# superxslam/SuperOdom

Measured on AMD Instinct MI355X. Metric: icp_registrations_per_sec, higher is better.
Workload: dtype f64

## Files before the change

superodom_amd/csrc/kernels.hip:

```cpp
#include <hip/hip_runtime.h>
#include <hip/hip_ext.h>

#include <cstddef>
#include <cstdlib>
#include <cstring>
#include <type_traits>

#ifdef SO_LM_STAMPS
#define SO_LM_STAMP(dbg, i) do { if (dbg) (dbg)[i] = wall_clock64(); } while (0)
#endif
#include "device_idioms.h"
#include "kernels.h"
#include "plane_fit.h"

namespace soicp {

#define SO_MATCH_SUCCESS 0
#define SO_MATCH_NOT_ENOUGH 1
#define SO_MATCH_TOO_FAR 2
#define SO_MATCH_BAD_PCA 3
#define SO_MATCH_INVALID 4
#define SO_MATCH_MSE 5
#define SO_MATCH_DROPPED 254
#define SO_MATCH_PENDING 255
// ... 1547 lines not shown
}
__device__ __forceinline__ void publish_state_to(DevState* dst, const DevState* st, unsigned long long seq, int tid, int nthreads) {
  if (!dst) return;
  __threadfence_block();
  __syncthreads();
  const unsigned long long* src = reinterpret_cast<const unsigned long long*>(st);
  unsigned long long* out = reinterpret_cast<unsigned long long*>(dst);
  constexpr int kWords = (int)(offsetof(DevState, seq) / 8);
  for (int i = tid; i < kWords; i += nthreads) out[i] = src[i];
  __threadfence_system();
  __syncthreads();
  if (tid == 0) __hip_atomic_store(&dst->seq, seq, __ATOMIC_RELEASE, __HIP_MEMORY_SCOPE_SYSTEM);
}

__device__ __forceinline__ void copy_words(double* dst, const double* src, int n_doubles, int tid, int nthreads) {
  for (int i = tid; i < n_doubles; i += nthreads) dst[i] = src[i];
}
static_assert(sizeof(LmState) % 8 == 0 && sizeof(LmSums) % 8 == 0, "controller state must be double-aligned");

constexpr int kPartStride = SO_SOLVE_BLOCKS;
static_assert(kEvalBlocks <= kPartStride && kFitBlocksMax <= kPartStride && kNAcc <= kSumsStride, "partials table");
constexpr int kRedStride = kNAcc + 2;

template <int CTRL>
__device__ __forceinline__ double dpp_f64(double v) {
  const int lo = __builtin_amdgcn_update_dpp(0, __double2loint(v), CTRL, 0xF, 0xF, false);
  const int hi = __builtin_amdgcn_update_dpp(0, __double2hiint(v), CTRL, 0xF, 0xF, false);
  return __hiloint2double(hi, lo);
}
__device__ __forceinline__ double swap32_add(double a, double b) {
  const auto lo = __builtin_amdgcn_permlane32_swap((unsigned)__double2loint(a), (unsigned)__double2loint(b), false, false);
  const auto hi = __builtin_amdgcn_permlane32_swap((unsigned)__double2hiint(a), (unsigned)__double2hiint(b), false, false);
  return __hiloint2double((int)hi[0], (int)lo[0]) + __hiloint2double((int)hi[1], (int)lo[1]);
}
__device__ __forceinline__ double swap16_add(double a, double b) {
  const auto lo = __builtin_amdgcn_permlane16_swap((unsigned)__double2loint(a), (unsigned)__double2loint(b), false, false);
  const auto hi = __builtin_amdgcn_permlane16_swap((unsigned)__double2hiint(a), (unsigned)__double2hiint(b), false, false);
  return __hiloint2double((int)hi[0], (int)lo[0]) + __hiloint2double((int)hi[1], (int)lo[1]);
}
template <int CTRL>
__device__ __forceinline__ double row_stage_add(double a, double b, bool up) {
  const double keep = up ? b : a, give = up ? a : b;
  return keep + dpp_f64<CTRL>(give);
}
__device__ __forceinline__ double wave_reduce_scatter(const double (&acc)[kNAcc]) {
  static_assert(kNAcc > 16 && kNAcc <= 32, "butterfly over 32 value slots");
  const int lane = (int)(threadIdx.x & 63u);
  double u[16], w[8], x[4], y[2];
#pragma unroll
  for (int a = 0; a < 16; ++a) u[a] = swap32_add(acc[a], (a + 16 < kNAcc) ? acc[a + 16] : 0.0);
#pragma unroll
  for (int a = 0; a < 8; ++a) w[a] = swap16_add(u[a], u[a + 8]);
  const bool b3 = (lane & 8) != 0, b2 = (lane & 4) != 0, b1 = (lane & 2) != 0;
#pragma unroll
  for (int a = 0; a < 4; ++a) x[a] = row_stage_add<0x128>(w[a], w[a + 4], b3);
#pragma unroll
  for (int a = 0; a < 2; ++a) y[a] = row_stage_add<0x141>(x[a], x[a + 2], b2);
  const double z = row_stage_add<0x4E>(y[0], y[1], b1);
  return z + dpp_f64<0xB1>(z);
}
__device__ __forceinline__ double wg_reduce(const double (&acc)[kNAcc], double (*part)[32], int tid) {
  const double t = wave_reduce_scatter(acc);
  const int lane = tid & 63, wave = tid >> 6;
  if (!(lane & 1) && (lane >> 1) < kNAcc) part[wave][lane >> 1] = t;
  __syncthreads();
  double tot = 0;
  if (tid < kNAcc) tot = ((part[0][tid] + part[1][tid]) + part[2][tid]) + part[3][tid];
  return tot;
}

__device__ __forceinline__ double reduce_records(double (*red)[kRedStride], double (*part)[32], int tid) {
  const int a = tid & 31, cch = tid >> 5;
  if (a < kNAcc) {
    double s = 0;
#pragma unroll 8
    for (int r = 0; r < 32; ++r) s += red[cch * 32 + r][a];
    part[cch][a] = s;
  }
  __syncthreads();
  double tot = 0;
  if (tid < kNAcc) {
#pragma unroll
    for (int cc = 0; cc < 8; ++cc) tot += part[cc][tid];
  }
  return tot;
}

struct EvalShared {
  double red[256][kRedStride];
  double part[8][32];
  double part_odd[8][32];
  LmSums sums;
  LmState S;
  LmCtl ctl;
  double pose[7];
  int more;
  int32_t lh[16];
  int32_t hpart[8][16];
  int reg_done;
  bool is_last;
  unsigned long long peer_seq;
};
struct CorrCache {
  double nx[2][256], ny[2][256], nz[2][256], nw[2][256], c[2][256];
  float px[2][256], py[2][256], pz[2][256];
};
enum { kPassNotLast = 0, kPassMore = 1, kPassDone = 2, kPassSums = 3 };

struct WgSpan { uint32_t vb0, vb1, V; bool ctl; };
template <bool FIT, bool PERSIST = false, bool PROF = false, bool BATCH = false, bool PEER = false>
__device__ __forceinline__ int eval_pass(int slot, int fuse_lm, const Pose& pose, const float* __restrict__ spx,
                                         const float* __restrict__ spy, const float* __restrict__ spz,
                                         const CorrBuffers& corr, DevState* __restrict__ st, const EvalParams& ep,
                                         double* __restrict__ partials, uint32_t* __restrict__ ticket,
                                         int32_t* __restrict__ hist, LmSums* __restrict__ out,
                                         const float4* __restrict__ mpts, const uint32_t* __restrict__ nbr5,
                                         const MatchParams& mp, EvalShared& sh, unsigned long long pass_tag = 0,
                                         CorrCache* cc = nullptr, u4v* hand = nullptr, unsigned long long want = 0,
                                         const WgSpan span = WgSpan{0, 0, 0, false}) {
  constexpr bool keep_state = PERSIST;
  double (*red)[kRedStride] = sh.red;
  double (*part)[32] = sh.part;
  LmSums& sh_sums = sh.sums;
  LmState& sh_S = sh.S;
  LmCtl& sh_ctl = sh.ctl;
  int& sh_more = sh.more;
  int32_t* lh = sh.lh;
  bool& is_last = sh.is_last;
  const int tid = threadIdx.x;
  static_assert(!BATCH || PERSIST, "batched hypotheses run in the persistent solve launch");
  const int abl = PROF ? ep.ablate : 0;
  const bool stamp = PROF && (abl & 128) != 0;
  const uint32_t V = BATCH ? span.V : gridDim.x;
  const uint32_t vb_begin = BATCH ? span.vb0 : blockIdx.x, vb_end = BATCH ? span.vb1 : blockIdx.x + 1u;
  const bool is_ctl = BATCH ? span.ctl : (blockIdx.x == 0);
  unsigned long long t_begin = 0, t_loop = 0, t_red = 0, t_ticket = 0, t_loaded = 0, t_sums = 0, t_lm = 0;
  if (stamp) t_begin = wall_clock64();
  if (FIT) {
    if (tid < 16) lh[tid] = 0;
    __syncthreads();
  }
  const uint32_t n_kept = (abl & 64) ? 0u : ep.n_queries;
  const uint32_t qs = ep.q_stride;
  double acc[kNAcc];
  const double qx = pose.q[0], qy = pose.q[1], qz = pose.q[2], qw = pose.q[3];
  const double tx = 2 * qx, ty = 2 * qy, tz = 2 * qz;
  const double twx = tx * qw, twy = ty * qw, twz = tz * qw, txx = tx * qx, txy = ty * qx, txz = tz * qx;
  const double tyy = ty * qy, tyz = tz * qy, tzz = tz * qz;
  const double R00 = 1 - (tyy + tzz), R01 = txy - twz, R02 = txz + twy;
  const double R10 = txy + twz, R11 = 1 - (txx + tzz), R12 = tyz - twx;
  const double R20 = txz - twy, R21 = tyz + twx, R22 = 1 - (txx + tyy);
  const ObsAxes axes = obs_axes(pose);
  const double inv_a2 = 1.0 / ep.a2, rho_out = (ep.variant == 0) ? ep.a2 / 6.0 : ep.a2 / 3.0;
  auto tail = [&](double px, double py, double pz, double wx, double wy, double wz, const double4& nd, double c) {
    const double r = SO_FMA(nd.x, wx, SO_FMA(nd.y, wy, SO_FMA(nd.z, wz, nd.w)));
    const double s = r * r;
    double rho0, rho1;
    if (s <= ep.a2) {
      const double v = 1.0 - s * inv_a2, v2 = v * v;
      rho0 = rho_out * (1.0 - v2 * v); rho1 = (ep.variant == 0) ? 0.5 * v2 : v2;
    } else {
      rho0 = rho_out; rho1 = 0;
    }
    const double w = c * rho1;
    const double m0 = SO_FMA(R00, nd.x, SO_FMA(R10, nd.y, R20 * nd.z));
    const double m1 = SO_FMA(R01, nd.x, SO_FMA(R11, nd.y, R21 * nd.z));
    const double m2 = SO_FMA(R02, nd.x, SO_FMA(R12, nd.y, R22 * nd.z));
    const double J[6] = {nd.x, nd.y, nd.z, SO_FMA(py, m2, -(pz * m1)), SO_FMA(pz, m0, -(px * m2)), SO_FMA(px, m1, -(py * m0))};
    acc[0] = SO_FMA(0.5 * c, rho0, acc[0]);
    acc[1] += 1.0;
    const double wr = w * r;
    int k = 8;
#pragma unroll
    for (int a = 0; a < 6; ++a) {
      acc[2 + a] = SO_FMA(J[a], wr, acc[2 + a]);
      const double wj = w * J[a];
#pragma unroll
      for (int b = a; b < 6; ++b) { acc[k] = SO_FMA(wj, J[b], acc[k]); ++k; }
    }
  };
  auto body = [&](const uint32_t j, int status, const float* nb, int trip) {
    if (!FIT && status != SO_MATCH_SUCCESS) return;
    if (FIT && status == SO_MATCH_DROPPED) return;
    const float fx = spx[(size_t)j * qs], fy = spy[(size_t)j * qs], fz = spz[(size_t)j * qs];
    const double px = (double)fx, py = (double)fy, pz = (double)fz;
    double wx, wy, wz;
    quat_rotate<double>(pose.q, px, py, pz, wx, wy, wz);
    wx += pose.t[0]; wy += pose.t[1]; wz += pose.t[2];
    double c;
    double4 nd;
    if (FIT) {
      if (PERSIST && !BATCH && trip >= 0) {
        cc->px[trip][tid] = fx; cc->py[trip][tid] = fy; cc->pz[trip][tid] = fz;
      }
      double fnd[4] = {0, 0, 0, 0}, fc = 0;
      int obs[3] = {0, 0, 0};
      if (status == SO_MATCH_PENDING) {
        const double pw[3] = {wx, wy, wz};
        if (PROF && (mp.ablate & (512 | 4096))) status = plane_fit5_reference(nb, pw, axes, mp.sq_max_dist_f, mp.max_point_dist, fnd, fc, obs, (mp.ablate & 512) != 0);
        else status = plane_fit5(nb, pw, axes, mp.sq_max_dist_f, mp.max_point_dist, fnd, fc, obs);
      }
      if (status != SO_MATCH_SUCCESS) { fc = 0; fnd[0] = fnd[1] = fnd[2] = fnd[3] = 0; }
      nd = make_double4(fnd[0], fnd[1], fnd[2], fnd[3]);
      c = fc;
      __builtin_nontemporal_store(nd.x, &corr.nd[j].x); __builtin_nontemporal_store(nd.y, &corr.nd[j].y);
      __builtin_nontemporal_store(nd.z, &corr.nd[j].z); __builtin_nontemporal_store(nd.w, &corr.nd[j].w);
      __builtin_nontemporal_store(c, &corr.coeff[j]); __builtin_nontemporal_store((uint8_t)status, &corr.status[j]);
      atomicAdd(&lh[status], 1);
      if (status == SO_MATCH_SUCCESS) { atomicAdd(&lh[7 + obs[0]], 1); atomicAdd(&lh[7 + obs[1]], 1); atomicAdd(&lh[7 + obs[2]], 1); }
      if (status != SO_MATCH_SUCCESS) return;
      if (PERSIST && !BATCH && trip >= 0) {
        cc->nx[trip][tid] = nd.x; cc->ny[trip][tid] = nd.y; cc->nz[trip][tid] = nd.z; cc->nw[trip][tid] = nd.w;
        cc->c[trip][tid] = c;
      }
    } else {
      c = corr.coeff[j];
      nd = corr.nd[j];
    }
    tail(px, py, pz, wx, wy, wz, nd, c);
  };
  double mine = 0;
  u4v* rec = reinterpret_cast<u4v*>(partials);
  const unsigned int tag = (unsigned int)pass_tag;
  struct Fetched { int st; double4 nd; double c; float x, y, z; };
  Fetched cur[2], nxt[2];
  auto fetch2 = [&](uint32_t vb_, Fetched (&o)[2]) {
#pragma unroll
    for (int q = 0; q < 2; ++q) {
      const uint32_t j = query_of(vb_, V, tid, (uint32_t)q);
      const uint32_t js = j < n_kept ? j : 0u;
      o[q].st = j < n_kept ? (int)corr.status[js] : (int)SO_MATCH_DROPPED;
      o[q].nd = corr.nd[js]; o[q].c = corr.coeff[js];
      o[q].x = spx[(size_t)js * qs]; o[q].y = spy[(size_t)js * qs]; o[q].z = spz[(size_t)js * qs];
    }
  };
  if (BATCH && !FIT && vb_begin < vb_end) fetch2(vb_begin, cur);
  for (uint32_t vb = vb_begin, trip_ = 0; BATCH ? (vb < vb_end) : (trip_ < 1u); ++vb, ++trip_) {
#pragma unroll
  for (int a = 0; a < kNAcc; ++a) acc[a] = 0;
  if (FIT) {
    if (PERSIST && !BATCH) { cc->c[0][tid] = -1.0; cc->c[1][tid] = -1.0; }
    bool first = true;
    if (BATCH) {
      for (uint32_t q = 0, j; (j = query_of(vb, V, tid, q)) < n_kept; ++q) {
        const int stq = corr.status[j];
        uint32_t iq[5];
#pragma unroll
        for (int t = 0; t < 5; ++t) iq[t] = nbr5[(size_t)5 * j + t];
        float nbq[15];
#pragma unroll
        for (int t = 0; t < 5; ++t) {
          const float4 a = mpts[stq == SO_MATCH_PENDING ? iq[t] : 0u];
          nbq[3 * t] = a.x; nbq[3 * t + 1] = a.y; nbq[3 * t + 2] = a.z;
        }
        body(j, stq, nbq, -1);
      }
    } else
    for (uint32_t q = 0, jA; (jA = query_of(vb, V, tid, q)) < n_kept; q += 2) {
      const uint32_t jB = query_of(vb, V, tid, q + 1u);
      const bool hasB = jB < n_kept;
      const uint32_t jBs = hasB ? jB : jA;
      const int stA = corr.status[jA];
      const int stB = hasB ? (int)corr.status[jBs] : SO_MATCH_NOT_ENOUGH;
      uint32_t iA[5], iB[5];
#pragma unroll
      for (int t = 0; t < 5; ++t) { iA[t] = nbr5[(size_t)5 * jA + t]; iB[t] = nbr5[(size_t)5 * jBs + t]; }
      float nbA[15], nbB[15];
#pragma unroll
      for (int t = 0; t < 5; ++t) {
        const float4 a = mpts[stA == SO_MATCH_PENDING ? iA[t] : 0u], b = mpts[stB == SO_MATCH_PENDING ? iB[t] : 0u];
        nbA[3 * t] = a.x; nbA[3 * t + 1] = a.y; nbA[3 * t + 2] = a.z;
        nbB[3 * t] = b.x; nbB[3 * t + 1] = b.y; nbB[3 * t + 2] = b.z;
      }
      body(jA, stA, nbA, first ? 0 : -1);
      if (hasB) body(jB, stB, nbB, first ? 1 : -1);
      first = false;
    }
  } else if (PERSIST && !BATCH) {
#pragma unroll
    for (int trip = 0; trip < 2; ++trip) {
      const double c = cc->c[trip][tid];
      const double4 nd = make_double4(cc->nx[trip][tid], cc->ny[trip][tid], cc->nz[trip][tid], cc->nw[trip][tid]);
      const double px = (double)cc->px[trip][tid], py = (double)cc->py[trip][tid], pz = (double)cc->pz[trip][tid];
      if (c >= 0.0) {
        double wx, wy, wz;
        quat_rotate<double>(pose.q, px, py, pz, wx, wy, wz);
        wx += pose.t[0]; wy += pose.t[1]; wz += pose.t[2];
        tail(px, py, pz, wx, wy, wz, nd, c);
      }
    }
    for (uint32_t q = 2, j; (j = query_of(vb, V, tid, q)) < n_kept; ++q) body(j, corr.status[j], nullptr, -1);
  } else if (BATCH) {
    if (vb + 1u < vb_end) fetch2(vb + 1u, nxt);
#pragma unroll
    for (int q = 0; q < 2; ++q)
      if (cur[q].st == SO_MATCH_SUCCESS) {
        const double px = (double)cur[q].x, py = (double)cur[q].y, pz = (double)cur[q].z;
        double wx, wy, wz;
        quat_rotate<double>(pose.q, px, py, pz, wx, wy, wz);
        wx += pose.t[0]; wy += pose.t[1]; wz += pose.t[2];
        tail(px, py, pz, wx, wy, wz, cur[q].nd, cur[q].c);
      }
    for (uint32_t q = 2, j; (j = query_of(vb, V, tid, q)) < n_kept; ++q) body(j, corr.status[j], nullptr, -1);
    cur[0] = nxt[0]; cur[1] = nxt[1];
  } else {
    for (uint32_t q = 0, j; (j = query_of(vb, V, tid, q)) < n_kept; ++q) body(j, corr.status[j], nullptr, -1);
  }
  if (stamp) t_loop = wall_clock64();
  mine = wg_reduce(acc, (BATCH && (trip_ & 1u)) ? sh.part_odd : part, tid);
  if (PERSIST) {
    static_assert(SO_SOLVE_BLOCKS == 256, "record table: 8 groups of 32 workgroups");
    static_assert(kNAcc <= kRecordChunksMax, "record table");
    if (FIT) __builtin_amdgcn_s_waitcnt(0x0F70);
    if (tid < kNAcc) {
      const unsigned long long b = (unsigned long long)__double_as_longlong(mine);
      const unsigned int extra = (FIT && tid < 16 && (!BATCH || vb + 1u == vb_end)) ? (unsigned int)lh[tid] : 0u;
      const u4v v = {(unsigned int)b, (unsigned int)(b >> 32), tag, extra};
      const uint32_t w = vb;
      store16_sc1(rec + ((w & 31u) * 8u + (w >> 5)) * kNAcc + tid, v);
    }
  }
  }
  if (PERSIST) {
    if (stamp) t_red = wall_clock64();
    if (!is_ctl) return kPassNotLast;
    constexpr int kPoll = 8 * kNAcc;
    const bool poller = tid < kPoll;
    const int g = poller ? tid / kNAcc : 0, a = poller ? tid - g * kNAcc : 0;
    const u4v* base = rec + (poller ? tid : 0);
    if (!BATCH) {
    u4v r[32];
    const unsigned long long t0 = wall_clock64();
    bool ok;
    for (;;) {
#pragma unroll
      for (int i = 0; i < 32; ++i)
        asm volatile("global_load_dwordx4 %0, %1, off sc1" : "=v"(r[i]) : "v"(base + (size_t)i * kPoll) : "memory");
      asm volatile("s_waitcnt vmcnt(0)"
                   : "+v"(r[0]), "+v"(r[1]), "+v"(r[2]), "+v"(r[3]), "+v"(r[4]), "+v"(r[5]), "+v"(r[6]), "+v"(r[7]), "+v"(r[8]), "+v"(r[9]),
                     "+v"(r[10]), "+v"(r[11]), "+v"(r[12]), "+v"(r[13]), "+v"(r[14]), "+v"(r[15]), "+v"(r[16]), "+v"(r[17]), "+v"(r[18]),
                     "+v"(r[19]), "+v"(r[20]), "+v"(r[21]), "+v"(r[22]), "+v"(r[23]), "+v"(r[24]), "+v"(r[25]), "+v"(r[26]), "+v"(r[27]),
                     "+v"(r[28])
                   :: "memory");
      asm volatile("" : "+v"(r[29]), "+v"(r[30]), "+v"(r[31]) :: "memory");
      ok = true;
#pragma unroll
      for (int i = 0; i < 32; ++i) ok = ok && (r[i].z == tag || (uint32_t)(32 * g + i) >= V);
      ok = ok || !poller;
      if (abl & 8192) { ok = false; break; }
      if (__ballot(!ok) == 0ull) break;
      if (wall_clock64() - t0 > ep.timeout_ticks) break;
    }
    if (!__syncthreads_and(ok ? 1 : 0)) return kPassNotLast;
    if (stamp) t_ticket = t_loaded = wall_clock64();
    {
      double sum = 0;
      int hsum = 0;
#pragma unroll
      for (int i = 0; i < 32; ++i) {
        const bool have = (uint32_t)(32 * g + i) < V;
        sum += have ? __longlong_as_double((long long)(((unsigned long long)r[i].y << 32) | r[i].x)) : 0.0;
        if (FIT) hsum += have ? (int)r[i].w : 0;
      }
      if (poller) {
        part[g][a] = sum;
        if (FIT && a < 16) sh.hpart[g][a] = hsum;
      }
    }
    } else {
      double sum = 0;
      int hsum = 0;
      bool ok = true;
      const unsigned long long t0 = wall_clock64();
      for (int i0 = 0; i0 < 32; i0 += 8) {
        u4v r[8];
        for (;;) {
#pragma unroll
          for (int k = 0; k < 8; ++k)
            asm volatile("global_load_dwordx4 %0, %1, off sc1" : "=v"(r[k]) : "v"(base + (size_t)(i0 + k) * kPoll) : "memory");
          asm volatile("s_waitcnt vmcnt(0)" : "+v"(r[0]), "+v"(r[1]), "+v"(r[2]), "+v"(r[3]), "+v"(r[4]), "+v"(r[5]), "+v"(r[6]), "+v"(r[7]) :: "memory");
          bool good = true;
#pragma unroll
          for (int k = 0; k < 8; ++k) good = good && (r[k].z == tag || (uint32_t)(32 * g + i0 + k) >= V);
          good = good || !poller;
          if (abl & 8192) good = false;
          if (__ballot(!good) == 0ull) break;
          if ((abl & 8192) || wall_clock64() - t0 > ep.timeout_ticks) { ok = ok && good; break; }
          __builtin_amdgcn_s_sleep(32);
        }
        if (__ballot(!ok) != 0ull) break;
#pragma unroll
        for (int k = 0; k < 8; ++k) {
          const bool have = (uint32_t)(32 * g + i0 + k) < V;
          sum += have ? __longlong_as_double((long long)(((unsigned long long)r[k].y << 32) | r[k].x)) : 0.0;
          if (FIT) hsum += have ? (int)r[k].w : 0;
        }
      }
      if (!__syncthreads_and(ok ? 1 : 0)) return kPassNotLast;
      if (poller) {
        part[g][a] = sum;
        if (FIT && a < 16) sh.hpart[g][a] = hsum;
      }
    }
    __syncthreads();
    double* o = reinterpret_cast<double*>(&sh_sums);
    if (tid < kNAcc) {
      double tot = 0;
#pragma unroll
      for (int cc8 = 0; cc8 < 8; ++cc8) tot += part[cc8][tid];
      o[tid] = tot;
    } else if (FIT && tid >= 32 && tid < 48) {
      int h = 0;
#pragma unroll
      for (int cc8 = 0; cc8 < 8; ++cc8) h += sh.hpart[cc8][tid - 32];
      o[kNAcc + (tid - 32)] = (double)h;
    }
    __syncthreads();
    if (PEER && ep.peer_world > 1) {
      const int nx = FIT ? (kNAcc + 16) : kNAcc;
      const unsigned int xtag = (unsigned int)(sh.peer_seq + 1ull);
      const int par = (int)(xtag & 1u);
      if (tid < nx) {
        const unsigned long long b = (unsigned long long)__double_as_longlong(o[tid]);
        const u4v v = {(unsigned int)b, (unsigned int)(b >> 32), xtag, (unsigned int)ep.peer_rank};
        for (int p = 0; p < ep.peer_world; ++p)
          store16_sys(reinterpret_cast<u4v*>(ep.peer_inbox[p]) + (size_t)(par * kPeerMaxWorld + ep.peer_rank) * kPeerChunks + tid, v);
      }
      const u4v* own = reinterpret_cast<const u4v*>(ep.peer_inbox[ep.peer_rank]) + (size_t)par * kPeerMaxWorld * kPeerChunks;
// ... 491 lines not shown
```

superodom_amd/csrc/plane_fit.h:

```cpp
#pragma once
#include "so_math.h"

namespace soicp {

#define SO_FIT_SUCCESS 0
#define SO_FIT_BAD_PCA 3
#define SO_FIT_INVALID 4
#define SO_FIT_MSE 5

#if defined(__HIP_DEVICE_COMPILE__)
#define SO_UNROLL _Pragma("unroll")
#define SO_UNROLL_NONE _Pragma("unroll 1")
#else
#define SO_UNROLL
#define SO_UNROLL_NONE
#endif

SO_HD double fit_div(double a, double b) {
#if defined(__HIP_DEVICE_COMPILE__)
  double r = __builtin_amdgcn_rcp(b);
  r = __builtin_fma(__builtin_fma(-b, r, 1.0), r, r);
  r = __builtin_fma(__builtin_fma(-b, r, 1.0), r, r);
  const double q = a * r;
  return __builtin_fma(__builtin_fma(-b, q, a), r, q);
#else
  return a / b;
#endif
}
SO_HD double fit_rsqrt(double x) {
#if defined(__HIP_DEVICE_COMPILE__)
  return rsqrt(x);
#else
  return 1.0 / sqrt(x);
#endif
}

struct ObsAxes { float ax[3][3]; };
SO_HD ObsAxes obs_axes(const Pose& pose) {
  ObsAxes o;
  const float qf[4] = {(float)pose.q[0], (float)pose.q[1], (float)pose.q[2], (float)pose.q[3]};
  quat_rotate<float>(qf, 1.f, 0.f, 0.f, o.ax[0][0], o.ax[0][1], o.ax[0][2]);
  quat_rotate<float>(qf, 0.f, 1.f, 0.f, o.ax[1][0], o.ax[1][1], o.ax[1][2]);
  quat_rotate<float>(qf, 0.f, 0.f, 1.f, o.ax[2][0], o.ax[2][1], o.ax[2][2]);
  return o;
}

SO_HD void eig3_sym_direct_adj(double a00, double a01, double a02, double a11, double a12, double a22, double ev[3], double nrm[3],
                               double adj[6], double& det_s, double& scale) {
  const double mx = fmax(fmax(fmax(fabs(a00), fabs(a11)), fabs(a22)), fmax(fmax(fabs(a01), fabs(a02)), fabs(a12)));
  scale = mx; det_s = 0.0;
  adj[0] = adj[1] = adj[2] = adj[3] = adj[4] = adj[5] = 0.0;
  if (!(mx > 0.0)) { ev[0] = ev[1] = ev[2] = 0.0; nrm[0] = 1.0; nrm[1] = 0.0; nrm[2] = 0.0; return; }
  const double is = fit_div(1.0, mx);
  a00 *= is; a01 *= is; a02 *= is; a11 *= is; a12 *= is; a22 *= is;
  const double c2 = a00 + a11 + a22;
  const double m00 = a11 * a22 - a12 * a12, m11 = a00 * a22 - a02 * a02, m22 = a00 * a11 - a01 * a01;
  const double c1 = m00 + m11 + m22;
  const double t01 = a01 * a22 - a12 * a02, t02 = a01 * a12 - a11 * a02;
  const double c0 = a00 * m00 - a01 * t01 + a02 * t02;
  adj[0] = m00; adj[1] = -t01; adj[2] = t02; adj[3] = m11; adj[4] = a01 * a02 - a00 * a12; adj[5] = m22;
  det_s = c0;
  double l = 0.0;
  SO_UNROLL_NONE
  for (int it = 0; it < 60; ++it) {
    const double f = ((-l + c2) * l - c1) * l + c0;
    const double df = (-3.0 * l + 2.0 * c2) * l - c1;
    if (!(df < 0.0) || !(f > 0.0)) break;
    const double step = fit_div(f, df);
    l -= step;
    if (!(-step > 4e-16)) break;
  }
  if (!(l > 0.0)) l = fmax(l, 0.0);
  const double sm = c2 - l, pr = c1 - l * sm;
  double disc = sm * sm - 4.0 * pr;
  disc = disc > 0.0 ? sqrt(disc) : 0.0;
  const double l2 = 0.5 * (sm + disc);
  const double l1 = (l2 > 0.0) ? fit_div(pr, l2) : 0.0;
  ev[0] = l * mx; ev[1] = l1 * mx; ev[2] = l2 * mx;
  const double r00 = a00 - l, r11 = a11 - l, r22 = a22 - l;
  const double x0 = a01 * a12 - a02 * r11, x1 = a02 * a01 - r00 * a12, x2 = r00 * r11 - a01 * a01;
  const double y0 = a01 * r22 - a02 * a12, y1 = a02 * a02 - r00 * r22, y2 = r00 * a12 - a01 * a02;
  const double z0 = r11 * r22 - a12 * a12, z1 = a12 * a02 - a01 * r22, z2 = a01 * a12 - r11 * a02;
  const double nx = x0 * x0 + x1 * x1 + x2 * x2, ny = y0 * y0 + y1 * y1 + y2 * y2, nz = z0 * z0 + z1 * z1 + z2 * z2;
  double v0 = x0, v1 = x1, v2 = x2, nn = nx;
  if (ny > nn) { v0 = y0; v1 = y1; v2 = y2; nn = ny; }
  if (nz > nn) { v0 = z0; v1 = z1; v2 = z2; nn = nz; }
  if (!(nn > 0.0)) { nrm[0] = 1.0; nrm[1] = 0.0; nrm[2] = 0.0; return; }
  const double inv = fit_rsqrt(nn);
  nrm[0] = v0 * inv; nrm[1] = v1 * inv; nrm[2] = v2 * inv;
}

template <bool AS_WRITTEN>
SO_HD void fit_observability(const double pw[3], const double ev[3], const double nrm[3], const ObsAxes& A, int& o0, int& o1, int& o2) {
  const float px = (float)pw[0], py = (float)pw[1], pz = (float)pw[2];
  const float nx = (float)nrm[0], ny = (float)nrm[1], nz = (float)nrm[2];
  const float cx = py * nz - pz * ny, cy = pz * nx - px * nz, cz = px * ny - py * nx;
  float rot[6], f[3];
  SO_UNROLL
  for (int a = 0; a < 3; ++a) {
    const float v = cx * A.ax[a][0] + cy * A.ax[a][1] + cz * A.ax[a][2];
    rot[2 * a] = v; rot[2 * a + 1] = -v;
    f[a] = fabsf(nx * A.ax[a][0] + ny * A.ax[a][1] + nz * A.ax[a][2]);
  }
  int b1 = 0;
  SO_UNROLL
  for (int a = 1; a < 6; ++a) if (rot[a] > rot[b1]) b1 = a;
  int b2 = -1;
  SO_UNROLL
  for (int a = 0; a < 6; ++a) if (a != b1 && (b2 < 0 || rot[a] > rot[b2])) b2 = a;
  int t1 = 0;
  if (f[1] > f[t1]) t1 = 1;
  if (f[2] > f[t1]) t1 = 2;
  const float fb = f[t1] * (1.0f - 9.5367431640625e-7f);
  const bool clear = (t1 == 0 || f[0] < fb) && (t1 == 1 || f[1] < fb) && (t1 == 2 || f[2] < fb);
  if (AS_WRITTEN || !(clear && ev[1] > 1.0001 * ev[0] && ev[0] > 0.0)) {
    const double l1 = sqrt(ev[2]), l2 = sqrt(ev[1]), l3 = sqrt(ev[0]);
    const double planar_2 = fit_div(l2 - l3, l1);
    const float psq = (float)(planar_2 * planar_2);
    const float tr[3] = {psq * f[0], psq * f[1], psq * f[2]};
    t1 = 0;
    if (tr[1] > tr[t1]) t1 = 1;
    if (tr[2] > tr[t1]) t1 = 2;
  }
  o0 = b1; o1 = b2; o2 = 6 + t1;
}

SO_HD int plane_fit5(const float nb[15], const double pw[3], const ObsAxes& axes, float sq_max_dist_f, double max_point_dist,
                     double nd[4], double& coeff, int obs[3], bool obs_as_written = false) {
  double mx = 0, my = 0, mz = 0;
  SO_UNROLL
  for (int j = 0; j < 5; ++j) { mx += (double)nb[3 * j]; my += (double)nb[3 * j + 1]; mz += (double)nb[3 * j + 2]; }
  mx = fit_div(mx, 5.0); my = fit_div(my, 5.0); mz = fit_div(mz, 5.0);
  double s00 = 0, s01 = 0, s02 = 0, s11 = 0, s12 = 0, s22 = 0;
  SO_UNROLL
  for (int j = 0; j < 5; ++j) {
    const double a = (double)nb[3 * j] - mx, b = (double)nb[3 * j + 1] - my, c = (double)nb[3 * j + 2] - mz;
    s00 += a * a; s01 += a * b; s02 += a * c; s11 += b * b; s12 += b * c; s22 += c * c;
  }
  double ev[3], nrm[3], adj[6], det_s, scale;
  eig3_sym_direct_adj(s00, s01, s02, s11, s12, s22, ev, nrm, adj, det_s, scale);
  if (ev[0] < 1e-6 || fit_div(ev[1], ev[2]) < 0.1) return SO_FIT_BAD_PCA;
  const double w0 = __builtin_fma(adj[0], mx, __builtin_fma(adj[1], my, adj[2] * mz));
  const double w1 = __builtin_fma(adj[1], mx, __builtin_fma(adj[3], my, adj[4] * mz));
  const double w2 = __builtin_fma(adj[2], mx, __builtin_fma(adj[4], my, adj[5] * mz));
  const double ww = __builtin_fma(w0, w0, __builtin_fma(w1, w1, w2 * w2));
  const double D = __builtin_fma(scale, det_s, 5.0 * __builtin_fma(w0, mx, __builtin_fma(w1, my, w2 * mz)));
  if (!(ww > 0.0) || !(D > 0.0) || !(D < 1.79e308)) return SO_FIT_INVALID;
  const double rs = fit_rsqrt(ww);
  const double n0 = -w0 * rs, n1 = -w1 * rs, n2 = -w2 * rs;
  const double d = (0.2 * D) * rs;
  double sum = 0;
  bool too_far = false;
  SO_UNROLL
  for (int j = 0; j < 5; ++j) {
    const double dist = fabs(n0 * (double)nb[3 * j] + n1 * (double)nb[3 * j + 1] + n2 * (double)nb[3 * j + 2] + d);
    too_far |= dist > max_point_dist;
    sum += dist;
  }
  if (too_far) return SO_FIT_MSE;
  const double mean_abs = fit_div(sum, 5.0);
  if (pw[0] * nrm[0] + pw[1] * nrm[1] + pw[2] * nrm[2] < 0) { nrm[0] = -nrm[0]; nrm[1] = -nrm[1]; nrm[2] = -nrm[2]; }
  if (obs_as_written) fit_observability<true>(pw, ev, nrm, axes, obs[0], obs[1], obs[2]);
  else fit_observability<false>(pw, ev, nrm, axes, obs[0], obs[1], obs[2]);
  coeff = 1.0 - sqrt(fit_div(mean_abs, (double)sq_max_dist_f));
  nd[0] = n0; nd[1] = n1; nd[2] = n2; nd[3] = d;
  return SO_FIT_SUCCESS;
}

SO_HD void jacobi_rot(double& app, double& aqq, double& apq, double& arp, double& arq,
                      double& v0p, double& v0q, double& v1p, double& v1q, double& v2p, double& v2q) {
  if (apq == 0.0) return;
  const double d = aqq - app, b2 = 2.0 * apq;
  const double t = (d >= 0 ? b2 : -b2) / (fabs(d) + sqrt(d * d + b2 * b2));
  const double c = fit_rsqrt(t * t + 1.0), s = t * c;
  app -= t * apq; aqq += t * apq; apq = 0.0;
  const double rp = c * arp - s * arq, rq = s * arp + c * arq;
  arp = rp; arq = rq;
  double a, b;
  a = c * v0p - s * v0q; b = s * v0p + c * v0q; v0p = a; v0q = b;
  a = c * v1p - s * v1q; b = s * v1p + c * v1q; v1p = a; v1q = b;
  a = c * v2p - s * v2q; b = s * v2p + c * v2q; v2p = a; v2q = b;
}

SO_HD void eig3_sym(double a00, double a01, double a02, double a11, double a12, double a22, double ev[3], double nrm[3]) {
  double v00 = 1, v01 = 0, v02 = 0, v10 = 0, v11 = 1, v12 = 0, v20 = 0, v21 = 0, v22 = 1;
  for (int sweep = 0; sweep < 16; ++sweep) {
    const double off = a01 * a01 + a02 * a02 + a12 * a12;
    const double dg = a00 * a00 + a11 * a11 + a22 * a22;
    if (off <= 1e-30 * dg || off == 0.0) break;
    jacobi_rot(a00, a11, a01, a02, a12, v00, v01, v10, v11, v20, v21);
    jacobi_rot(a00, a22, a02, a01, a12, v00, v02, v10, v12, v20, v22);
    jacobi_rot(a11, a22, a12, a01, a02, v01, v02, v11, v12, v21, v22);
  }
  double e0 = a00, e1 = a11, e2 = a22;
  double n0 = v00, n1 = v10, n2 = v20;
  if (e1 < e0 && e1 <= e2) { n0 = v01; n1 = v11; n2 = v21; }
  else if (e2 < e0 && e2 < e1) { n0 = v02; n1 = v12; n2 = v22; }
  double t;
  if (e0 > e1) { t = e0; e0 = e1; e1 = t; }
  if (e1 > e2) { t = e1; e1 = e2; e2 = t; }
  if (e0 > e1) { t = e0; e0 = e1; e1 = t; }
  ev[0] = e0; ev[1] = e1; ev[2] = e2;
  nrm[0] = n0; nrm[1] = n1; nrm[2] = n2;
}

SO_HD bool plane_ls5(const float nb[15], double x[3]) {
  double A[3][5], b[5];
  int perm[3] = {0, 1, 2};
  SO_UNROLL
  for (int i = 0; i < 5; ++i) {
    A[0][i] = (double)nb[3 * i]; A[1][i] = (double)nb[3 * i + 1]; A[2][i] = (double)nb[3 * i + 2];
    b[i] = -1.0;
  }
  SO_UNROLL
  for (int k = 0; k < 3; ++k) {
    double nrm[3] = {0, 0, 0};
    SO_UNROLL
    for (int j = k; j < 3; ++j) {
      double s = 0;
      SO_UNROLL
      for (int i = k; i < 5; ++i) s += A[j][i] * A[j][i];
      nrm[j] = s;
    }
    int piv = k;
    double best = nrm[k];
    SO_UNROLL
    for (int j = k + 1; j < 3; ++j)
      if (nrm[j] > best) { best = nrm[j]; piv = j; }
    SO_UNROLL
    for (int j = k + 1; j < 3; ++j)
      if (piv == j) {
        SO_UNROLL
        for (int i = 0; i < 5; ++i) { const double t = A[k][i]; A[k][i] = A[j][i]; A[j][i] = t; }
        const int t = perm[k]; perm[k] = perm[j]; perm[j] = t;
      }
    double alpha = sqrt(best);
    if (alpha != 0.0) {
      if (A[k][k] > 0) alpha = -alpha;
      double v[5];
      double vn2 = 0;
      SO_UNROLL
      for (int i = k; i < 5; ++i) v[i] = A[k][i];
      v[k] -= alpha;
      SO_UNROLL
      for (int i = k; i < 5; ++i) vn2 += v[i] * v[i];
      if (vn2 != 0.0) {
        SO_UNROLL
        for (int j = k + 1; j < 3; ++j) {
          double dot = 0;
          SO_UNROLL
          for (int i = k; i < 5; ++i) dot += v[i] * A[j][i];
          const double f = fit_div(2.0 * dot, vn2);
          SO_UNROLL
          for (int i = k; i < 5; ++i) A[j][i] -= f * v[i];
        }
        double dot = 0;
        SO_UNROLL
        for (int i = k; i < 5; ++i) dot += v[i] * b[i];
        const double f = fit_div(2.0 * dot, vn2);
        SO_UNROLL
        for (int i = k; i < 5; ++i) b[i] -= f * v[i];
        A[k][k] = alpha;
      }
    }
  }
  const double y2 = fit_div(b[2], A[2][2]);
  const double y1 = fit_div(b[1] - A[2][1] * y2, A[1][1]);
  const double y0 = fit_div(b[0] - A[1][0] * y1 - A[2][0] * y2, A[0][0]);
  SO_UNROLL
  for (int a = 0; a < 3; ++a) x[a] = (perm[0] == a) ? y0 : ((perm[1] == a) ? y1 : y2);
  return isfinite(x[0]) && isfinite(x[1]) && isfinite(x[2]);
}

SO_HD int plane_fit5_reference(const float nb[15], const double pw[3], const ObsAxes& axes, float sq_max_dist_f, double max_point_dist,
                               double nd[4], double& coeff, int obs[3], bool jacobi_eig) {
  double mx = 0, my = 0, mz = 0;
  SO_UNROLL
  for (int j = 0; j < 5; ++j) { mx += (double)nb[3 * j]; my += (double)nb[3 * j + 1]; mz += (double)nb[3 * j + 2]; }
  mx = fit_div(mx, 5.0); my = fit_div(my, 5.0); mz = fit_div(mz, 5.0);
  double s00 = 0, s01 = 0, s02 = 0, s11 = 0, s12 = 0, s22 = 0;
  SO_UNROLL
  for (int j = 0; j < 5; ++j) {
    const double a = (double)nb[3 * j] - mx, b = (double)nb[3 * j + 1] - my, c = (double)nb[3 * j + 2] - mz;
    s00 += a * a; s01 += a * b; s02 += a * c; s11 += b * b; s12 += b * c; s22 += c * c;
  }
  double ev[3], nrm[3];
  if (jacobi_eig) eig3_sym(s00, s01, s02, s11, s12, s22, ev, nrm);
  else {
    double adj[6], det_s, scale;
    eig3_sym_direct_adj(s00, s01, s02, s11, s12, s22, ev, nrm, adj, det_s, scale);
  }
  if (ev[0] < 1e-6 || fit_div(ev[1], ev[2]) < 0.1) return SO_FIT_BAD_PCA;
  double x[3];
  if (!plane_ls5(nb, x)) return SO_FIT_INVALID;
  const double nn = sqrt(x[0] * x[0] + x[1] * x[1] + x[2] * x[2]);
  const double d = fit_div(1.0, nn);
  const double n0 = fit_div(x[0], nn), n1 = fit_div(x[1], nn), n2 = fit_div(x[2], nn);
  double sum = 0;
  bool too_far = false;
  SO_UNROLL
  for (int j = 0; j < 5; ++j) {
    const double dist = fabs(n0 * (double)nb[3 * j] + n1 * (double)nb[3 * j + 1] + n2 * (double)nb[3 * j + 2] + d);
    too_far |= dist > max_point_dist;
    sum += dist;
  }
  if (too_far) return SO_FIT_MSE;
  const double mean_abs = fit_div(sum, 5.0);
  if (pw[0] * nrm[0] + pw[1] * nrm[1] + pw[2] * nrm[2] < 0) { nrm[0] = -nrm[0]; nrm[1] = -nrm[1]; nrm[2] = -nrm[2]; }
  fit_observability<true>(pw, ev, nrm, axes, obs[0], obs[1], obs[2]);
  coeff = 1.0 - sqrt(fit_div(mean_abs, (double)sq_max_dist_f));
  nd[0] = n0; nd[1] = n1; nd[2] = n2; nd[3] = d;
  return SO_FIT_SUCCESS;
}

#undef SO_UNROLL
#undef SO_UNROLL_NONE

}
```

Measured before the change: 7126.

## Fit two query planes jointly per thread with paired-lane plane fitting

Replaces the two sequential per-query body calls in the FIT path with a body_pair routine. It runs a two-wide plane fit (PCA via a direct cubic eigen solve with Newton iteration) on both queries at once using a D2 pair type, so independent instruction streams can be interleaved. It also splits the Jacobian accumulation into a term computation and an add step so both queries compute their terms before accumulating. The cost is more register pressure and extra computation on dead or non-pending lanes, and the fit may not match the original plane_fit path exactly.

```diff
diff --git a/superodom_amd/csrc/kernels.hip b/superodom_amd/csrc/kernels.hip
--- a/superodom_amd/csrc/kernels.hip
+++ b/superodom_amd/csrc/kernels.hip
@@ -1723,7 +1723,8 @@
   const double R20 = txz - twy, R21 = tyz + twx, R22 = 1 - (txx + tyy);
   const ObsAxes axes = obs_axes(pose);
   const double inv_a2 = 1.0 / ep.a2, rho_out = (ep.variant == 0) ? ep.a2 / 6.0 : ep.a2 / 3.0;
-  auto tail = [&](double px, double py, double pz, double wx, double wy, double wz, const double4& nd, double c) {
+  struct TailTerms { double J[6], w, wr, c, rho0; };
+  auto tail_terms = [&](double px, double py, double pz, double wx, double wy, double wz, const double4& nd, double c) {
     const double r = SO_FMA(nd.x, wx, SO_FMA(nd.y, wy, SO_FMA(nd.z, wz, nd.w)));
     const double s = r * r;
     double rho0, rho1;
@@ -1737,18 +1738,22 @@
     const double m0 = SO_FMA(R00, nd.x, SO_FMA(R10, nd.y, R20 * nd.z));
     const double m1 = SO_FMA(R01, nd.x, SO_FMA(R11, nd.y, R21 * nd.z));
     const double m2 = SO_FMA(R02, nd.x, SO_FMA(R12, nd.y, R22 * nd.z));
-    const double J[6] = {nd.x, nd.y, nd.z, SO_FMA(py, m2, -(pz * m1)), SO_FMA(pz, m0, -(px * m2)), SO_FMA(px, m1, -(py * m0))};
-    acc[0] = SO_FMA(0.5 * c, rho0, acc[0]);
+    return TailTerms{{nd.x, nd.y, nd.z, SO_FMA(py, m2, -(pz * m1)), SO_FMA(pz, m0, -(px * m2)), SO_FMA(px, m1, -(py * m0))}, w, w * r, c, rho0};
+  };
+  auto tail_add = [&](const TailTerms& t) {
+    acc[0] = SO_FMA(0.5 * t.c, t.rho0, acc[0]);
     acc[1] += 1.0;
-    const double wr = w * r;
     int k = 8;
 #pragma unroll
     for (int a = 0; a < 6; ++a) {
-      acc[2 + a] = SO_FMA(J[a], wr, acc[2 + a]);
-      const double wj = w * J[a];
-#pragma unroll
-      for (int b = a; b < 6; ++b) { acc[k] = SO_FMA(wj, J[b], acc[k]); ++k; }
-    }
+      acc[2 + a] = SO_FMA(t.J[a], t.wr, acc[2 + a]);
+      const double wj = t.w * t.J[a];
+#pragma unroll
+      for (int b = a; b < 6; ++b) { acc[k] = SO_FMA(wj, t.J[b], acc[k]); ++k; }
+    }
+  };
+  auto tail = [&](double px, double py, double pz, double wx, double wy, double wz, const double4& nd, double c) {
+    tail_add(tail_terms(px, py, pz, wx, wy, wz, nd, c));
   };
   auto body = [&](const uint32_t j, int status, const float* nb, int trip) {
     if (!FIT && status != SO_MATCH_SUCCESS) return;
@@ -1790,6 +1795,54 @@
     }
     tail(px, py, pz, wx, wy, wz, nd, c);
   };
+  auto body_pair = [&](const uint32_t jA, const uint32_t jB, int stA, int stB, bool hasB, const float* nbA, const float* nbB, bool first) {
+    const bool liveA = stA != SO_MATCH_DROPPED, liveB = hasB && stB != SO_MATCH_DROPPED;
+    const float fxA = spx[(size_t)jA * qs], fyA = spy[(size_t)jA * qs], fzA = spz[(size_t)jA * qs];
+    const float fxB = spx[(size_t)jB * qs], fyB = spy[(size_t)jB * qs], fzB = spz[(size_t)jB * qs];
+    const double pxA = (double)fxA, pyA = (double)fyA, pzA = (double)fzA, pxB = (double)fxB, pyB = (double)fyB, pzB = (double)fzB;
+    double pwA[3], pwB[3];
+    quat_rotate<double>(pose.q, pxA, pyA, pzA, pwA[0], pwA[1], pwA[2]);
+    pwA[0] += pose.t[0]; pwA[1] += pose.t[1]; pwA[2] += pose.t[2];
+    pwB[0] = pwB[1] = pwB[2] = 0.0;
+    if (liveB) {
+      quat_rotate<double>(pose.q, pxB, pyB, pzB, pwB[0], pwB[1], pwB[2]);
+      pwB[0] += pose.t[0]; pwB[1] += pose.t[1]; pwB[2] += pose.t[2];
+    }
+    if (PERSIST && first) {
+      cc->px[0][tid] = fxA; cc->py[0][tid] = fyA; cc->pz[0][tid] = fzA;
+      cc->px[1][tid] = fxB; cc->py[1][tid] = fyB; cc->pz[1][tid] = fzB;
+    }
+    int status[2] = {stA, stB}, obsA[3] = {0, 0, 0}, obsB[3] = {0, 0, 0};
+    double fndA[4] = {0, 0, 0, 0}, fndB[4] = {0, 0, 0, 0}, fc[2] = {0, 0};
+    plane_fit5_x2(nbA, nbB, pwA, pwB, axes, mp.sq_max_dist_f, mp.max_point_dist,
+                  B2{liveA && stA == SO_MATCH_PENDING, liveB && stB == SO_MATCH_PENDING}, status, fndA, fndB, fc, obsA, obsB);
+    const bool okA = liveA && status[0] == SO_MATCH_SUCCESS, okB = liveB && status[1] == SO_MATCH_SUCCESS;
+    const double4 ndA = okA ? make_double4(fndA[0], fndA[1], fndA[2], fndA[3]) : make_double4(0, 0, 0, 0);
+    const double4 ndB = okB ? make_double4(fndB[0], fndB[1], fndB[2], fndB[3]) : make_double4(0, 0, 0, 0);
+    const double cA = okA ? fc[0] : 0.0, cB = okB ? fc[1] : 0.0;
+    if (liveA) {
+      __builtin_nontemporal_store(ndA.x, &corr.nd[jA].x); __builtin_nontemporal_store(ndA.y, &corr.nd[jA].y);
+      __builtin_nontemporal_store(ndA.z, &corr.nd[jA].z); __builtin_nontemporal_store(ndA.w, &corr.nd[jA].w);
+      __builtin_nontemporal_store(cA, &corr.coeff[jA]); __builtin_nontemporal_store((uint8_t)status[0], &corr.status[jA]);
+      atomicAdd(&lh[status[0]], 1);
+    }
+    if (liveB) {
+      __builtin_nontemporal_store(ndB.x, &corr.nd[jB].x); __builtin_nontemporal_store(ndB.y, &corr.nd[jB].y);
+      __builtin_nontemporal_store(ndB.z, &corr.nd[jB].z); __builtin_nontemporal_store(ndB.w, &corr.nd[jB].w);
+      __builtin_nontemporal_store(cB, &corr.coeff[jB]); __builtin_nontemporal_store((uint8_t)status[1], &corr.status[jB]);
+      atomicAdd(&lh[status[1]], 1);
+    }
+    if (okA) { atomicAdd(&lh[7 + obsA[0]], 1); atomicAdd(&lh[7 + obsA[1]], 1); atomicAdd(&lh[7 + obsA[2]], 1); }
+    if (okB) { atomicAdd(&lh[7 + obsB[0]], 1); atomicAdd(&lh[7 + obsB[1]], 1); atomicAdd(&lh[7 + obsB[2]], 1); }
+    if (PERSIST && first) {
+      if (okA) { cc->nx[0][tid] = ndA.x; cc->ny[0][tid] = ndA.y; cc->nz[0][tid] = ndA.z; cc->nw[0][tid] = ndA.w; cc->c[0][tid] = cA; }
+      if (okB) { cc->nx[1][tid] = ndB.x; cc->ny[1][tid] = ndB.y; cc->nz[1][tid] = ndB.z; cc->nw[1][tid] = ndB.w; cc->c[1][tid] = cB; }
+    }
+    const TailTerms tA = tail_terms(pxA, pyA, pzA, pwA[0], pwA[1], pwA[2], ndA, cA);
+    const TailTerms tB = tail_terms(pxB, pyB, pzB, pwB[0], pwB[1], pwB[2], ndB, cB);
+    if (okA) tail_add(tA);
+    if (okB) tail_add(tB);
+  };
   double mine = 0;
   u4v* rec = reinterpret_cast<u4v*>(partials);
   const unsigned int tag = (unsigned int)pass_tag;
@@ -1843,8 +1896,10 @@
         nbA[3 * t] = a.x; nbA[3 * t + 1] = a.y; nbA[3 * t + 2] = a.z;
         nbB[3 * t] = b.x; nbB[3 * t + 1] = b.y; nbB[3 * t + 2] = b.z;
       }
-      body(jA, stA, nbA, first ? 0 : -1);
-      if (hasB) body(jB, stB, nbB, first ? 1 : -1);
+      if (PROF && (mp.ablate & (512 | 4096))) {
+        body(jA, stA, nbA, first ? 0 : -1);
+        if (hasB) body(jB, stB, nbB, first ? 1 : -1);
+      } else body_pair(jA, jBs, stA, stB, hasB, nbA, nbB, first);
       first = false;
     }
   } else if (PERSIST && !BATCH) {
diff --git a/superodom_amd/csrc/plane_fit.h b/superodom_amd/csrc/plane_fit.h
--- a/superodom_amd/csrc/plane_fit.h
+++ b/superodom_amd/csrc/plane_fit.h
@@ -165,6 +165,148 @@
   coeff = 1.0 - sqrt(fit_div(mean_abs, (double)sq_max_dist_f));
   nd[0] = n0; nd[1] = n1; nd[2] = n2; nd[3] = d;
   return SO_FIT_SUCCESS;
+}
+
+struct D2 { double a, b; };
+struct B2 { bool a, b; };
+SO_HD D2 d2(double x) { return D2{x, x}; }
+SO_HD D2 operator+(D2 x, D2 y) { return D2{x.a + y.a, x.b + y.b}; }
+SO_HD D2 operator-(D2 x, D2 y) { return D2{x.a - y.a, x.b - y.b}; }
+SO_HD D2 operator*(D2 x, D2 y) { return D2{x.a * y.a, x.b * y.b}; }
+SO_HD D2 operator*(double k, D2 x) { return D2{k * x.a, k * x.b}; }
+SO_HD D2 operator-(D2 x) { return D2{-x.a, -x.b}; }
+SO_HD D2& operator+=(D2& x, D2 y) { x.a += y.a; x.b += y.b; return x; }
+SO_HD D2 fma2(D2 x, D2 y, D2 z) { return D2{__builtin_fma(x.a, y.a, z.a), __builtin_fma(x.b, y.b, z.b)}; }
+SO_HD D2 abs2(D2 x) { return D2{fabs(x.a), fabs(x.b)}; }
+SO_HD D2 max2(D2 x, D2 y) { return D2{fmax(x.a, y.a), fmax(x.b, y.b)}; }
+SO_HD D2 sqrt2(D2 x) { return D2{sqrt(x.a), sqrt(x.b)}; }
+SO_HD D2 rsqrt2(D2 x) { return D2{fit_rsqrt(x.a), fit_rsqrt(x.b)}; }
+SO_HD D2 sel2(B2 m, D2 x, D2 y) { return D2{m.a ? x.a : y.a, m.b ? x.b : y.b}; }
+SO_HD D2 div2(D2 a, D2 b) {
+#if defined(__HIP_DEVICE_COMPILE__)
+  D2 r = D2{__builtin_amdgcn_rcp(b.a), __builtin_amdgcn_rcp(b.b)};
+  r = fma2(fma2(-b, r, d2(1.0)), r, r);
+  r = fma2(fma2(-b, r, d2(1.0)), r, r);
+  const D2 q = a * r;
+  return fma2(fma2(-b, q, a), r, q);
+#else
+  return D2{a.a / b.a, a.b / b.b};
+#endif
+}
+
+SO_HD void eig3_sym_direct_adj_x2(D2 a00, D2 a01, D2 a02, D2 a11, D2 a12, D2 a22, D2 ev[3], D2 nrm[3], D2 adj[6], D2& det_s, D2& scale, B2& live) {
+  D2 mx = max2(max2(max2(abs2(a00), abs2(a11)), abs2(a22)), max2(max2(abs2(a01), abs2(a02)), abs2(a12)));
+  live = B2{mx.a > 0.0, mx.b > 0.0};
+  mx = sel2(live, mx, d2(1.0));
+  scale = mx;
+  const D2 is = div2(d2(1.0), mx);
+  a00 = a00 * is; a01 = a01 * is; a02 = a02 * is; a11 = a11 * is; a12 = a12 * is; a22 = a22 * is;
+  const D2 c2 = a00 + a11 + a22;
+  const D2 m00 = a11 * a22 - a12 * a12, m11 = a00 * a22 - a02 * a02, m22 = a00 * a11 - a01 * a01;
+  const D2 c1 = m00 + m11 + m22;
+  const D2 t01 = a01 * a22 - a12 * a02, t02 = a01 * a12 - a11 * a02;
+  const D2 c0 = a00 * m00 - a01 * t01 + a02 * t02;
+  adj[0] = m00; adj[1] = -t01; adj[2] = t02; adj[3] = m11; adj[4] = a01 * a02 - a00 * a12; adj[5] = m22;
+  det_s = c0;
+  D2 l = d2(0.0);
+  B2 go = B2{true, true};
+  SO_UNROLL_NONE
+  for (int it = 0; it < 60; ++it) {
+    const D2 f = ((-l + c2) * l - c1) * l + c0;
+    const D2 df = (-3.0 * l + 2.0 * c2) * l - c1;
+    go.a = go.a && (df.a < 0.0) && (f.a > 0.0); go.b = go.b && (df.b < 0.0) && (f.b > 0.0);
+    const D2 step = div2(f, df);
+    l = sel2(go, l - step, l);
+    go.a = go.a && (-step.a > 4e-16); go.b = go.b && (-step.b > 4e-16);
+    if (!(go.a || go.b)) break;
+  }
+  l = sel2(B2{l.a > 0.0, l.b > 0.0}, l, max2(l, d2(0.0)));
+  const D2 sm = c2 - l, pr = c1 - l * sm;
+  D2 disc = sm * sm - 4.0 * pr;
+  disc = sel2(B2{disc.a > 0.0, disc.b > 0.0}, sqrt2(disc), d2(0.0));
+  const D2 l2 = 0.5 * (sm + disc);
+  const D2 l1 = sel2(B2{l2.a > 0.0, l2.b > 0.0}, div2(pr, l2), d2(0.0));
+  ev[0] = l * mx; ev[1] = l1 * mx; ev[2] = l2 * mx;
+  const D2 r00 = a00 - l, r11 = a11 - l, r22 = a22 - l;
+  const D2 x0 = a01 * a12 - a02 * r11, x1 = a02 * a01 - r00 * a12, x2 = r00 * r11 - a01 * a01;
+  const D2 y0 = a01 * r22 - a02 * a12, y1 = a02 * a02 - r00 * r22, y2 = r00 * a12 - a01 * a02;
+  const D2 z0 = r11 * r22 - a12 * a12, z1 = a12 * a02 - a01 * r22, z2 = a01 * a12 - r11 * a02;
+  const D2 nx = x0 * x0 + x1 * x1 + x2 * x2, ny = y0 * y0 + y1 * y1 + y2 * y2, nz = z0 * z0 + z1 * z1 + z2 * z2;
+  D2 v0 = x0, v1 = x1, v2 = x2, nn = nx;
+  B2 m = B2{ny.a > nn.a, ny.b > nn.b};
+  v0 = sel2(m, y0, v0); v1 = sel2(m, y1, v1); v2 = sel2(m, y2, v2); nn = sel2(m, ny, nn);
+  m = B2{nz.a > nn.a, nz.b > nn.b};
+  v0 = sel2(m, z0, v0); v1 = sel2(m, z1, v1); v2 = sel2(m, z2, v2); nn = sel2(m, nz, nn);
+  m = B2{nn.a > 0.0, nn.b > 0.0};
+  const D2 inv = rsqrt2(nn);
+  nrm[0] = sel2(m, v0 * inv, d2(1.0)); nrm[1] = sel2(m, v1 * inv, d2(0.0)); nrm[2] = sel2(m, v2 * inv, d2(0.0));
+}
+
+SO_HD void plane_fit5_x2(const float nbA[15], const float nbB[15], const double pwA[3], const double pwB[3], const ObsAxes& axes,
+                         float sq_max_dist_f, double max_point_dist, B2 run, int status[2], double ndA[4], double ndB[4],
+                         double coeff[2], int obsA[3], int obsB[3]) {
+  D2 nb[15];
+  SO_UNROLL
+  for (int j = 0; j < 15; ++j) nb[j] = D2{(double)nbA[j], (double)nbB[j]};
+  D2 mx = d2(0), my = d2(0), mz = d2(0);
+  SO_UNROLL
+  for (int j = 0; j < 5; ++j) { mx += nb[3 * j]; my += nb[3 * j + 1]; mz += nb[3 * j + 2]; }
+  mx = div2(mx, d2(5.0)); my = div2(my, d2(5.0)); mz = div2(mz, d2(5.0));
+  D2 s00 = d2(0), s01 = d2(0), s02 = d2(0), s11 = d2(0), s12 = d2(0), s22 = d2(0);
+  SO_UNROLL
+  for (int j = 0; j < 5; ++j) {
+    const D2 a = nb[3 * j] - mx, b = nb[3 * j + 1] - my, c = nb[3 * j + 2] - mz;
+    s00 += a * a; s01 += a * b; s02 += a * c; s11 += b * b; s12 += b * c; s22 += c * c;
+  }
+  D2 ev[3], nrm[3], adj[6], det_s, scale;
+  B2 live;
+  eig3_sym_direct_adj_x2(s00, s01, s02, s11, s12, s22, ev, nrm, adj, det_s, scale, live);
+  const D2 ratio = div2(ev[1], ev[2]);
+  int fitA = (!live.a || ev[0].a < 1e-6 || ratio.a < 0.1) ? SO_FIT_BAD_PCA : SO_FIT_SUCCESS;
+  int fitB = (!live.b || ev[0].b < 1e-6 || ratio.b < 0.1) ? SO_FIT_BAD_PCA : SO_FIT_SUCCESS;
+  const D2 w0 = fma2(adj[0], mx, fma2(adj[1], my, adj[2] * mz));
+  const D2 w1 = fma2(adj[1], mx, fma2(adj[3], my, adj[4] * mz));
+  const D2 w2 = fma2(adj[2], mx, fma2(adj[4], my, adj[5] * mz));
+  const D2 ww = fma2(w0, w0, fma2(w1, w1, w2 * w2));
+  const D2 D = fma2(scale, det_s, 5.0 * fma2(w0, mx, fma2(w1, my, w2 * mz)));
+  if (fitA == SO_FIT_SUCCESS && (!(ww.a > 0.0) || !(D.a > 0.0) || !(D.a < 1.79e308))) fitA = SO_FIT_INVALID;
+  if (fitB == SO_FIT_SUCCESS && (!(ww.b > 0.0) || !(D.b > 0.0) || !(D.b < 1.79e308))) fitB = SO_FIT_INVALID;
+  const D2 rs = rsqrt2(ww);
+  const D2 n0 = -w0 * rs, n1 = -w1 * rs, n2 = -w2 * rs;
+  const D2 d = (0.2 * D) * rs;
+  D2 sum = d2(0);
+  B2 too_far = B2{false, false};
+  SO_UNROLL
+  for (int j = 0; j < 5; ++j) {
+    const D2 dist = abs2(n0 * nb[3 * j] + n1 * nb[3 * j + 1] + n2 * nb[3 * j + 2] + d);
+    too_far.a |= dist.a > max_point_dist; too_far.b |= dist.b > max_point_dist;
+    sum += dist;
+  }
+  if (fitA == SO_FIT_SUCCESS && too_far.a) fitA = SO_FIT_MSE;
+  if (fitB == SO_FIT_SUCCESS && too_far.b) fitB = SO_FIT_MSE;
+  const D2 mean_abs = div2(sum, d2(5.0));
+  const D2 pA = D2{pwA[0], pwB[0]}, pB = D2{pwA[1], pwB[1]}, pC = D2{pwA[2], pwB[2]};
+  const D2 side = pA * nrm[0] + pB * nrm[1] + pC * nrm[2];
+  const B2 flip = B2{side.a < 0, side.b < 0};
+  nrm[0] = sel2(flip, -nrm[0], nrm[0]); nrm[1] = sel2(flip, -nrm[1], nrm[1]); nrm[2] = sel2(flip, -nrm[2], nrm[2]);
+  const D2 co = d2(1.0) - sqrt2(div2(mean_abs, d2((double)sq_max_dist_f)));
+  const bool okA = run.a && fitA == SO_FIT_SUCCESS, okB = run.b && fitB == SO_FIT_SUCCESS;
+  int oA[3] = {0, 0, 0}, oB[3] = {0, 0, 0};
+  if (okA) {
+    const double n[3] = {nrm[0].a, nrm[1].a, nrm[2].a}, e[3] = {ev[0].a, ev[1].a, ev[2].a};
+    fit_observability<false>(pwA, e, n, axes, oA[0], oA[1], oA[2]);
+  }
+  if (okB) {
+    const double n[3] = {nrm[0].b, nrm[1].b, nrm[2].b}, e[3] = {ev[0].b, ev[1].b, ev[2].b};
+    fit_observability<false>(pwB, e, n, axes, oB[0], oB[1], oB[2]);
+  }
+  if (run.a) status[0] = fitA;
+  if (run.b) status[1] = fitB;
+  ndA[0] = okA ? n0.a : ndA[0]; ndA[1] = okA ? n1.a : ndA[1]; ndA[2] = okA ? n2.a : ndA[2]; ndA[3] = okA ? d.a : ndA[3];
+  ndB[0] = okB ? n0.b : ndB[0]; ndB[1] = okB ? n1.b : ndB[1]; ndB[2] = okB ? n2.b : ndB[2]; ndB[3] = okB ? d.b : ndB[3];
+  coeff[0] = okA ? co.a : coeff[0]; coeff[1] = okB ? co.b : coeff[1];
+  obsA[0] = okA ? oA[0] : obsA[0]; obsA[1] = okA ? oA[1] : obsA[1]; obsA[2] = okA ? oA[2] : obsA[2];
+  obsB[0] = okB ? oB[0] : obsB[0]; obsB[1] = okB ? oB[1] : obsB[1]; obsB[2] = okB ? oB[2] : obsB[2];
 }
 
 SO_HD void jacobi_rot(double& app, double& aqq, double& apq, double& arp, double& arq,
```

Result: no change. 7137 (median of 2 runs) (+0.2%).
